# aszepieniec/stark-anatomy

Hardware: AMD Instinct MI355X
Metric: ntt_field_elements_per_sec (higher is better)
Workload: dtype u128; 1 GPU; ntt_fwd_inv_2^20_1gpu; log2n=20, parallelism=single, passes_per_transform=2

## Files before the change

### stark-anatomy_amd/csrc/core.h

```cpp
#pragma once
#include <hip/hip_runtime.h>
#include <dlfcn.h>
#include <cstdio>
#include <cstdlib>
#include <cstring>
#include <algorithm>
#include <atomic>
#include <chrono>
#include <cerrno>
#include <thread>
#include <sys/random.h>
#include <deque>
#include <functional>
#include <future>
#include <map>
#include <mutex>
#include <string>
#include <tuple>
#include <vector>

#pragma GCC visibility push(default)
#include "../../include/starkcore.h"
#pragma GCC visibility pop
#include "ntt_plan.h"

namespace sc { struct FoldIn; }
using namespace sc;

struct sc_vec {
    Fe* d;
    uint64_t n;
    bool owned = true;
};
struct sc_later {
    int slot;
    uint64_t seq;
    hipStream_t st;
};
struct sc_merkle {
    uint64_t* d_levels;
    uint64_t N;
    int logN;
    int slot = -1;
    uint64_t seq = 0;
    hipStream_t st = nullptr;
    bool have_root = false;
    bool lazy = false;
    uint8_t root[64] = {};
};

struct sc_merkle_forest {
    uint64_t* d_levels;
    uint64_t N, count;
    int logN;
    uint64_t* h_roots = nullptr;
    Fe* d_cm = nullptr;
    hipEvent_t done = nullptr;
    hipStream_t st = nullptr;
    bool have_roots = false;
};

namespace sci {

struct DevBuf {
    void* p = nullptr;
    size_t bytes = 0;
};

struct PlanKey {
    int logn;
    uint64_t lo, hi;
    bool operator<(const PlanKey& o) const { return std::tie(logn, lo, hi) < std::tie(o.logn, o.lo, o.hi); }
};
struct PlanTables {
    Fe* mt = nullptr;
    int mt_log = 0;
    Fe* tl = nullptr;
    Fe* th = nullptr;
    Fe* th_ninv = nullptr;
    struct Direct { int logA, logR; bool scaled; Fe* d; };
    std::vector<Direct> direct;
    uint64_t last_use = 0;
};
struct OuterKey {
    uint64_t lo, hi, order, len, batch, col_base;
    int ninv;
    bool operator<(const OuterKey& o) const { return std::tie(lo, hi, order, len, batch, col_base, ninv) < std::tie(o.lo, o.hi, o.order, o.len, o.batch, o.col_base, o.ninv); }
};
struct OuterTable {
    Fe* d = nullptr;
    uint64_t last_use = 0;
};
struct PowKey {
    uint64_t lo, hi, hi_count;
    bool operator<(const PowKey& o) const { return std::tie(lo, hi, hi_count) < std::tie(o.lo, o.hi, o.hi_count); }
};
struct PowTables {
    Fe* lo = nullptr;
    Fe* hi = nullptr;
    uint64_t last_use = 0;
};

struct Ctx {
    bool init = false;
    int device = -1;
    hipStream_t stream = nullptr;
    std::string err;
    NttTuning tuning;
    std::map<PlanKey, PlanTables> plans;
    std::map<PowKey, PowTables> pows;
    std::map<OuterKey, OuterTable> outers;
    uint64_t tick = 0;
    bool foreign_streams = false;
    int small_divisor_direct = 1;
    int div_cols_launch_log = 26;
    int tree_cols_launch_log = 26;
    int eval_chunk_log = 8;
    int eval_points_across_min = 32;
    int eval_across_min_products_log = 26;
    int rescue_tree_split_max_nodes = -1;
    int div_cols_chunk = 0;
    std::vector<hipStream_t> seen_streams;
    DevBuf scratch[8];
    std::map<hipStream_t, DevBuf> ntt_work;
    std::map<hipStream_t, DevBuf> ntt_flags;
    int fast_fixups = 1;
    int num_cus = 256;
    int xcd_remap = 1;
    int fixed_shapes = 1;
    int prio_balance = -1;
    int wave_local = 1;
    unsigned long long* trace = nullptr;
    int forest_four_lane_wgs = 256;
    int merkle_big_nlev = 2;
    int fri_tail = -1;
    int fri_tail_stall = -1;
    size_t verify_stage_bytes = 64ull << 20;
    uint8_t* root_slots = nullptr;
    uint8_t* later_words = nullptr;
    uint64_t root_seq = 0;
    std::vector<int> free_root_slots;
};
constexpr int ROOT_SLOTS = 256;
constexpr size_t ROOT_SLOT_BYTES = 128;
constexpr size_t LATER_WORD_BYTES = 128;
constexpr long SPIN_POLLS = 40000000;

struct PendingFree {
    void* p;
    size_t bytes;
    std::vector<hipEvent_t> evs;
};
#define HIPCHK(expr)                                                                                          \
    do {                                                                                                      \
        hipError_t _e = (expr);                                                                               \
        if (_e != hipSuccess) return fail(SC_ERR_HIP, std::string(#expr) + ": " + hipGetErrorString(_e));     \
    } while (0)

#define SCCHK(expr)              \
    do {                         \
        int _rc = (expr);        \
        if (_rc != SC_OK) return _rc; \
    } while (0)

struct NttOpts {
    uint64_t in_limit = ~0ull;
    const PowTables* coset = nullptr;
    uint32_t cols = 1;
    uint64_t col_stride_in = 0;
};
constexpr uint64_t COLS_ELEMS_PER_LAUNCH = 1ull << 26;
constexpr uint64_t SMALL_DIVISOR = 8;

constexpr uint64_t FUSE_MAX_W = 1ull << 17;

enum BuildMode { BUILD_SYNC = 0, BUILD_ASYNC = 1, BUILD_NOROOT = 2 };

extern Ctx g;
extern std::mutex g_mu;
extern hipStream_t g_comm_stream_for_free;
extern std::future<void> g_rand_worker;
extern size_t g_rand_prefetched;
extern std::multimap<size_t, void*> g_pool;
extern size_t g_pool_bytes, g_pool_cap;
extern std::deque<PendingFree> g_pending;
extern std::vector<hipEvent_t> g_event_pool;

void reap_pending(bool block);
hipError_t pool_alloc(void** p, size_t bytes);
void pool_free(void* p, size_t bytes);
void pool_clear();
hipEvent_t event_get();
int fail(int code, const std::string& msg);
int ensure_init();
int grow_buffer(DevBuf& b, size_t bytes, void** out);
inline int scratch(int slot, size_t bytes, void** out) { return grow_buffer(g.scratch[slot], bytes, out); }
int check_root(Fe root, uint64_t n);
int build_pow_table(Fe** out, uint64_t count, Fe base_m, uint64_t step, Fe scale_m, hipStream_t st);
void free_plans();
int evict_outer_tables();
int get_plan(Fe root, int logn, bool need_ninv, hipStream_t st, PlanTables** out);
inline NttTables tables_of(const PlanTables& t) {
    NttTables tb;
    tb.mt = t.mt; tb.mt_log = t.mt_log; tb.tl = t.tl; tb.th = t.th;
    return tb;
}
int get_pow(Fe base, uint64_t count, hipStream_t st, PowTables** out);
int plan_batched_direct(NttPlanDesc& d, BatchKind kind, int loglen, int logbatch, PlanTables* pt, const Fe* in, Fe* work, Fe* out, BatchExtras ex, hipStream_t st, bool* ok);
int run_plan(NttPlanDesc& d, hipStream_t st);
int ntt_device(const Fe* d_in, Fe* d_out, int logn, Fe root, bool inverse_scale, const NttOpts& o, hipStream_t st);
Fe root_inverse(Fe root, uint64_t n);
int ntt_any(const Fe* d_in, Fe* d_out, uint64_t n, Fe root, bool inverse, const NttOpts& o, hipStream_t st);
int upload(void* d, const void* h, size_t bytes, hipStream_t st);
int download(void* h, const void* d, size_t bytes, hipStream_t st);
int pointwise_div_device(const Fe* a, const Fe* b, Fe* out, uint64_t n, hipStream_t st);
int pointwise_div_enqueue(const Fe* a, const Fe* b, Fe* out, uint64_t n, hipStream_t st, uint32_t* flag);
int gather_device(const Fe* v, const uint64_t* d_idx, uint64_t k, Fe* d_out, hipStream_t st);
int read_small_polled(const void* d_src, size_t bytes, hipStream_t st, void* host_out);
bool upload_small(void* d_dst, const void* host, size_t bytes, hipStream_t st);

int merkle_climb(uint64_t* levels, uint64_t N, int lvl, hipStream_t st, volatile uint64_t* host = nullptr, uint64_t seq = 0, bool* published = nullptr);
int merkle_finish(uint64_t* levels, uint64_t width, hipStream_t st);
int root_slot_get();
int merkle_build_device(const Fe* d_elems, uint64_t N, uint8_t root_out[64], sc_merkle** tree, hipStream_t st, BuildMode mode = BUILD_SYNC, const FoldIn* fold = nullptr);
int merkle_root_wait(sc_merkle* t, bool from_free = false);
void root_poll_unlocked(std::unique_lock<std::mutex>& lk, const sc_merkle* t);
int fold_prepare(const Fe* d_in, uint64_t N, Fe alpha, Fe offset, Fe omega, Fe* d_out, hipStream_t st, FoldIn* f);
int fold_device(const Fe* d_in, uint64_t N, Fe alpha, Fe offset, Fe omega, Fe* d_out, hipStream_t st);
int fold_and_build(const Fe* d_in, uint64_t N, Fe alpha, Fe offset, Fe omega, Fe* d_out, sc_merkle** tree, hipStream_t st);
int fold_constants(uint64_t N, Fe offset, Fe omega, hipStream_t st, PowTables** pw_out, Fe* i2o_m_out);
int host_pool_get(size_t bytes, void** out);
int host_pool_put(void* p);
bool host_pool_holds(const void* p, size_t bytes);
int verify_stage_buffer(size_t bytes, uint8_t** out);

Fe canonical_root(int logn);
Fe ninv_scaled(int logn, int j);
int ntt_cols(const Fe* in, Fe* out, int loglen, int logbatch, bool inverse, hipStream_t st);

constexpr size_t SEEN_STREAMS = 8;
inline hipStream_t pick_stream(void* s) {
    if (s && (hipStream_t)s != g.stream) {
        g.foreign_streams = true;
        hipStream_t st = (hipStream_t)s;
        if (g.seen_streams.size() <= SEEN_STREAMS && std::find(g.seen_streams.begin(), g.seen_streams.end(), st) == g.seen_streams.end())
            g.seen_streams.push_back(st);
    }
    return s ? (hipStream_t)s : g.stream;
}
inline void release_after_streams(void* p, size_t bytes) {
    if (!p) return;
    if (g.seen_streams.size() > SEEN_STREAMS) {
        (void)hipDeviceSynchronize();
        g.seen_streams.clear();
        pool_free(p, bytes);
        return;
    }
    PendingFree f{p, bytes, {}};
    auto mark = [&](hipStream_t st) -> bool {
        if (hipStreamQuery(st) == hipSuccess) return true;
        (void)hipGetLastError();
        hipEvent_t e = event_get();
        if (!e) { (void)hipStreamSynchronize(st); (void)hipGetLastError(); return true; }
        if (hipEventRecord(e, st) != hipSuccess) { (void)hipGetLastError(); g_event_pool.push_back(e); return false; }
        f.evs.push_back(e);
        return true;
    };
    if (g.stream) (void)mark(g.stream);
    if (g_comm_stream_for_free) (void)mark(g_comm_stream_for_free);
    for (size_t i = 0; i < g.seen_streams.size();) {
        if (mark(g.seen_streams[i])) ++i;
        else g.seen_streams.erase(g.seen_streams.begin() + i);
    }
    if (f.evs.empty()) { pool_free(p, bytes); return; }
    g_pending.push_back(std::move(f));
    reap_pending(false);
}
inline Fe fe_from(const uint64_t v[2]) { return Fe{v[0], v[1]}; }
// ... 30 lines not shown
```

### stark-anatomy_amd/csrc/core.hip

```cpp
#include "core.h"


template <int LOGE> struct PassThreads { static constexpr int value = LOGE >= 4 ? 256 : (LOGE == 3 ? 512 : 1024); };

template <int LOGE>
__global__ void __launch_bounds__(PassThreads<LOGE>::value) ntt_pass_kernel(const PassParams P, uint32_t ntiles, int xcd_remap) {
    extern __shared__ __attribute__((aligned(16))) unsigned char smem_raw[];
    Fe* lds = reinterpret_cast<Fe*>(smem_raw);
    uint32_t wg = blockIdx.x, colbits = 0;
    if (P.col_enable) { colbits = (wg >> P.col_tiles_log) << P.col_tiles_log; wg -= colbits; }
    uint32_t tile = wg;
    if (xcd_remap) tile = (wg & 7u) * (ntiles >> 3) + (wg >> 3);
    tile |= colbits;
    Fe* tw = lds + (1u << (P.logR + P.logC));
    tile_twiddles_to_lds(P, P.logR, threadIdx.x, blockDim.x, tw);
    __syncthreads();
    const int nrounds = (P.logR + LOGE - 1) / LOGE;
    int sh = P.logR;
    for (int r = 0; r < nrounds; ++r) {
        const int s = (r == 0) ? (P.logR - LOGE * (nrounds - 1)) : LOGE;
        sh -= s;
        ntt_round_dispatch<LOGE>(P, s, sh, r == 0, tile, threadIdx.x, lds, tw);
        if (r + 1 < nrounds) __syncthreads();
    }
}

constexpr int TRACE_STAMPS = 16;
template <int LOGE, int GLR, int GLC, bool TRACE, bool ALT = false>
__global__ void __launch_bounds__(1 << (GLR + GLC - LOGE)) ntt_pass_kernel_fixed(const PassParams P, uint32_t ntiles, int xcd_remap, int wave_local) {
    extern __shared__ __attribute__((aligned(16))) unsigned char smem_raw[];
    Fe* lds = reinterpret_cast<Fe*>(smem_raw);
    unsigned long long* trow = nullptr;
    if constexpr (TRACE) {
        if (P.trace) {
            trow = P.trace + ((size_t)blockIdx.x * (blockDim.x >> 6) + (threadIdx.x >> 6)) * TRACE_STAMPS;
            if ((threadIdx.x & 63u) == 0) { trow[0] = __builtin_amdgcn_s_memtime(); trow[15] = __builtin_amdgcn_s_memrealtime(); }
        }
    }
    uint32_t wg = blockIdx.x, colbits = 0;
    if (P.col_enable) { colbits = (wg >> P.col_tiles_log) << P.col_tiles_log; wg -= colbits; }
    uint32_t tile = wg;
    if (xcd_remap) tile = (wg & 7u) * (ntiles >> 3) + (wg >> 3);
    tile |= colbits;
    Fe* tw = lds + (1u << (GLR + GLC));
    auto stamp = [&](int i) {
        if constexpr (TRACE) {
            if (trow) {
                if (i == 2) __builtin_amdgcn_s_waitcnt(0);
                if ((threadIdx.x & 63u) == 0 && i < 13) trow[i] = __builtin_amdgcn_s_memtime();
            }
        }
    };
    auto sync = [] { __syncthreads(); };
    auto wsync = [] { __builtin_amdgcn_fence(__ATOMIC_RELEASE, "wavefront"); __builtin_amdgcn_wave_barrier(); __builtin_amdgcn_fence(__ATOMIC_ACQUIRE, "wavefront"); };
    FixedRounds<LOGE, GLR, GLC, 0, ALT>::run(P, tile, threadIdx.x, lds, tw, sync, wsync, stamp, wave_local != 0);
    if constexpr (TRACE) {
        if (trow && (threadIdx.x & 63u) == 0) { __builtin_amdgcn_s_waitcnt(0); trow[14] = __builtin_amdgcn_s_memtime(); trow[13] = __builtin_amdgcn_s_memrealtime(); }
    }
}

template <int GLR, int GLC>
__device__ __forceinline__ uint32_t fixed8_tile(const PassParams& P, uint32_t index, uint32_t ntiles, int xcd_remap) {
    uint32_t wg = index, colbits = 0;
    if (P.col_enable) { colbits = (wg >> P.col_tiles_log) << P.col_tiles_log; wg -= colbits; }
    uint32_t tile = wg;
    if (xcd_remap) tile = (wg & 7u) * (ntiles >> 3) + (wg >> 3);
    return tile | colbits;
}
template <int GLR, int GLC>
__global__ void __launch_bounds__(1 << (GLR + GLC - 3)) __attribute__((amdgpu_waves_per_eu(4)))
ntt_pass_kernel_fixed8(const PassParams P, uint32_t ntiles, int xcd_remap, int wave_local, uint32_t* flags) {
    extern __shared__ __attribute__((aligned(16))) unsigned char smem_raw[];
    Fe* lds = reinterpret_cast<Fe*>(smem_raw);
    const uint32_t tile = fixed8_tile<GLR, GLC>(P, blockIdx.x, ntiles, xcd_remap);
    Fe* tw = lds + (1u << (GLR + GLC));
    auto stamp = [](int) {};
    auto sync = [] { __syncthreads(); };
    auto wsync = [] { __builtin_amdgcn_fence(__ATOMIC_RELEASE, "wavefront"); __builtin_amdgcn_wave_barrier(); __builtin_amdgcn_fence(__ATOMIC_ACQUIRE, "wavefront"); };
    rare_t rare = 0;
    FixedRounds<3, GLR, GLC, 0, false, true>::run(P, tile, threadIdx.x, lds, tw, sync, wsync, stamp, wave_local != 0, rare);
    if (rare_any(rare)) Round<3, 3, GLR, GLC>::store_word_at(flags + blockIdx.x, 0u, 1u);
}

template <int GLR, int GLC>
__global__ void __launch_bounds__(1 << (GLR + GLC - 3)) __attribute__((amdgpu_waves_per_eu(4)))
ntt_pass_redo8_kernel(const PassParams P, uint32_t ntiles, int xcd_remap, int wave_local, uint32_t* flags, int all) {
    extern __shared__ __attribute__((aligned(16))) unsigned char smem_raw[];
    if (!all && flags[blockIdx.x] == 0) return;
    Fe* lds = reinterpret_cast<Fe*>(smem_raw);
    Fe* tw = lds + (1u << (GLR + GLC));
    auto stamp = [](int) {};
    auto sync = [] { __syncthreads(); };
    auto wsync = [] { __builtin_amdgcn_fence(__ATOMIC_RELEASE, "wavefront"); __builtin_amdgcn_wave_barrier(); __builtin_amdgcn_fence(__ATOMIC_ACQUIRE, "wavefront"); };
    FixedRounds<3, GLR, GLC, 0, false>::run(P, fixed8_tile<GLR, GLC>(P, blockIdx.x, ntiles, xcd_remap), threadIdx.x, lds, tw, sync, wsync, stamp, wave_local != 0);
    if (!all) __syncthreads();
    if (threadIdx.x == 0) flags[blockIdx.x] = 0;
}

__global__ void __launch_bounds__(256) pow_table_kernel(Fe* out, uint64_t count, Fe base_m, uint64_t step, Fe scale_m) {
    uint64_t i = (uint64_t)blockIdx.x * blockDim.x + threadIdx.x;
    if (i < count) out[i] = pow_table_entry(base_m, i, step, scale_m);
}

__global__ void __launch_bounds__(256) twiddle_table_kernel(Fe* out, int logB, uint64_t count, uint64_t scale_exp, const Fe* __restrict__ tl, const Fe* __restrict__ th) {
    uint64_t i = (uint64_t)blockIdx.x * blockDim.x + threadIdx.x;
    if (i >= count) return;
    uint64_t k = i >> logB, b = i & ((1ull << logB) - 1);
    out[i] = pow2level(tl, th, b * k * scale_exp);
}

__global__ void __launch_bounds__(256) pointwise_mul_kernel(const Fe* __restrict__ a, const Fe* __restrict__ b, Fe* __restrict__ out, uint64_t n) {
    uint64_t i = (uint64_t)blockIdx.x * blockDim.x + threadIdx.x;
    if (i < n) out[i] = fe_mul(a[i], b[i]);
}

template <int K>
__global__ void __launch_bounds__(256) pointwise_div_kernel(const Fe* __restrict__ a, const Fe* __restrict__ b, Fe* __restrict__ out, uint64_t n, uint32_t* flag) {
    const uint64_t nthreads = (uint64_t)gridDim.x * blockDim.x;
    const uint64_t t = (uint64_t)blockIdx.x * blockDim.x + threadIdx.x;
    Fe bm[K], pre[K];
    Fe acc = fe_mont_one();
    bool zero = false;
#pragma unroll
    for (int k = 0; k < K; ++k) {
        uint64_t i = t + (uint64_t)k * nthreads;
        Fe v = (i < n) ? b[i] : fe_one();
        zero |= fe_is_zero(v);
        bm[k] = to_mont(v);
        pre[k] = acc;
        acc = mont_mul(acc, bm[k]);
    }
    if (zero) atomicOr(flag, 1u);
    Fe inv = mont_inv(acc);
#pragma unroll
    for (int k = K - 1; k >= 0; --k) {
        uint64_t i = t + (uint64_t)k * nthreads;
        Fe ik = mont_mul(inv, pre[k]);
        inv = mont_mul(inv, bm[k]);
        if (i < n) out[i] = mont_mul(a[i], ik);
    }
}

__global__ void __launch_bounds__(256) short_poly_coset_kernel(const Fe* __restrict__ b, uint32_t nb, Fe off_m, const Fe* __restrict__ tl, const Fe* __restrict__ th, Fe* __restrict__ out, uint64_t order) {
    const uint64_t i = (uint64_t)blockIdx.x * blockDim.x + threadIdx.x;
    if (i >= order) return;
    const Fe x_m = mont_mul(off_m, pow2level(tl, th, i));
    Fe acc = b[nb - 1];
    for (uint32_t k = nb - 1; k-- > 0;) acc = fe_add(mont_mul(acc, x_m), b[k]);
    out[i] = acc;
}

__global__ void __launch_bounds__(256) scale_pow_kernel(const Fe* __restrict__ in, Fe* __restrict__ out, uint64_t n, const Fe* __restrict__ lo, const Fe* __restrict__ hi) {
    uint64_t i = (uint64_t)blockIdx.x * blockDim.x + threadIdx.x;
    if (i < n) out[i] = mont_mul(in[i], pow2level(lo, hi, i));
}

__global__ void __launch_bounds__(256) scale_slab_kernel(const Fe* __restrict__ in, Fe* __restrict__ out, uint64_t rows, int logcols, uint64_t row_len, uint64_t col_base,
                                                         const Fe* __restrict__ lo, const Fe* __restrict__ hi) {
    uint64_t t = (uint64_t)blockIdx.x * blockDim.x + threadIdx.x;
    if (t >= (rows << logcols)) return;
    uint64_t r = t >> logcols, c = t & ((1ull << logcols) - 1);
    out[t] = mont_mul(in[t], pow2level(lo, hi, r * row_len + col_base + c));
}

__global__ void __launch_bounds__(256) axpy_shift_kernel(Fe* __restrict__ acc, const Fe* __restrict__ src, uint64_t n_src, uint64_t shift, Fe w_m) {
    uint64_t j = (uint64_t)blockIdx.x * blockDim.x + threadIdx.x;
    if (j >= n_src) return;
    acc[shift + j] = fe_add(acc[shift + j], mont_mul(src[j], w_m));
}

constexpr int DEGREE_PER_THREAD = 4;
constexpr unsigned DEGREE_MAX_BLOCKS = 2048;
constexpr int DEGREE_SLOTS = 8;
__global__ void __launch_bounds__(256) vec_degree_kernel(const Fe* __restrict__ v, uint64_t n, long long* out) {
    const uint64_t step = (uint64_t)gridDim.x * (256 * DEGREE_PER_THREAD);
    long long best = -1;
    for (uint64_t base = (uint64_t)blockIdx.x * (256 * DEGREE_PER_THREAD) + threadIdx.x; base - threadIdx.x < n; base += step) {
        Fe x[DEGREE_PER_THREAD];
#pragma unroll
        for (int k = 0; k < DEGREE_PER_THREAD; ++k) {
            const uint64_t i = base + 256u * k;
            x[k] = i < n ? v[i] : Fe{0, 0};
        }
#pragma unroll
        for (int k = 0; k < DEGREE_PER_THREAD; ++k) {
            const unsigned long long lanes = __ballot(!fe_is_zero(x[k]));
            if (lanes) best = (long long)(base - (threadIdx.x & 63u) + 256u * k + (63 - __clzll((long long)lanes)));
        }
    }
    __shared__ long long wave_best[4];
    if ((threadIdx.x & 63u) == 0) wave_best[threadIdx.x >> 6] = best;
    __syncthreads();
    if (threadIdx.x == 0) {
        long long m = wave_best[0];
#pragma unroll
        for (int w = 1; w < 4; ++w) m = wave_best[w] > m ? wave_best[w] : m;
        if (m >= 0) atomicMax(out + (blockIdx.x & (DEGREE_SLOTS - 1)), m);
    }
}
__global__ void __launch_bounds__(256) vec_degree_cols_kernel(const Fe* __restrict__ v, uint64_t n, uint64_t ld, uint32_t per_col, long long* out) {
    const uint64_t col = blockIdx.x / per_col;
    const uint32_t part = blockIdx.x - (uint32_t)col * per_col;
    const Fe* __restrict__ w = v + col * ld;
    const uint64_t step = (uint64_t)per_col * (256 * DEGREE_PER_THREAD);
    long long best = -1;
    for (uint64_t base = (uint64_t)part * (256 * DEGREE_PER_THREAD) + threadIdx.x; base - threadIdx.x < n; base += step) {
        Fe x[DEGREE_PER_THREAD];
#pragma unroll
        for (int k = 0; k < DEGREE_PER_THREAD; ++k) {
            const uint64_t i = base + 256u * k;
            x[k] = i < n ? w[i] : Fe{0, 0};
        }
#pragma unroll
        for (int k = 0; k < DEGREE_PER_THREAD; ++k) {
            const unsigned long long lanes = __ballot(!fe_is_zero(x[k]));
            if (lanes) best = (long long)(base - (threadIdx.x & 63u) + 256u * k + (63 - __clzll((long long)lanes)));
        }
    }
    __shared__ long long wave_best[4];
    if ((threadIdx.x & 63u) == 0) wave_best[threadIdx.x >> 6] = best;
    __syncthreads();
    if (threadIdx.x == 0) {
        long long m = wave_best[0];
#pragma unroll
        for (int k = 1; k < 4; ++k) m = wave_best[k] > m ? wave_best[k] : m;
        if (m >= 0) atomicMax(out + col, m);
    }
}
static int degree_read(void* fl, hipStream_t st, long long* deg) {
    long long slots[DEGREE_SLOTS];
    SCCHK(read_small_polled(fl, sizeof slots, st, slots));
    long long m = -1;
    for (int i = 0; i < DEGREE_SLOTS; ++i) m = slots[i] > m ? slots[i] : m;
    *deg = m;
// ... 206 lines not shown
    if (const char* sd = getenv("STARKCORE_DEVICE")) dev = atoi(sd) % n;
    HIPCHK(hipSetDevice(dev));
    HIPCHK(hipStreamCreateWithFlags(&g.stream, hipStreamNonBlocking));
    { int cus = 0; if (hipDeviceGetAttribute(&cus, hipDeviceAttributeMultiprocessorCount, dev) == hipSuccess && cus > 0) g.num_cus = cus; }
    { size_t free_b = 0, total_b = 0; if (hipMemGetInfo(&free_b, &total_b) == hipSuccess && total_b) g_pool_cap = total_b / 4; else (void)hipGetLastError(); }
    if (const char* lws = getenv("LOCAL_WORLD_SIZE")) { const int per_dev = (atoi(lws) + n - 1) / n; if (per_dev > 1) g_pool_cap /= (size_t)per_dev; }
    if (const char* cap = getenv("STARKCORE_POOL_CAP_MB")) g_pool_cap = (size_t)atoll(cap) << 20;
    g.device = dev;
    g.init = true;
    return SC_OK;
}

int grow_buffer(DevBuf& b, size_t bytes, void** out) {
    if (b.bytes < bytes) {
        if (b.p) { HIPCHK(hipDeviceSynchronize()); HIPCHK(hipFree(b.p)); b.p = nullptr; b.bytes = 0; }
        size_t want = bytes < (1u << 20) ? (1u << 20) : bytes;
        HIPCHK(hipMalloc(&b.p, want));
        b.bytes = want;
    }
    *out = b.p;
    return SC_OK;
}

int check_root(Fe root, uint64_t n) {
    if (fe_ge_p(root)) return fail(SC_ERR_BAD_ARG, "root is not a canonical residue");
    Fe rm = to_mont(root);
    Fe one = fe_mont_one();
    Fe half = mont_pow(rm, n / 2);
    Fe full = mont_mul(half, half);
    if (!fe_eq(full, one)) return fail(SC_ERR_ROOT_ORDER, "primitive root must be nth root of unity, where n is len(values)");
    if (fe_eq(half, one)) return fail(SC_ERR_ROOT_NOT_PRIMITIVE, "primitive root is not primitive nth root of unity, where n is len(values)");
    return SC_OK;
}

int build_pow_table(Fe** out, uint64_t count, Fe base_m, uint64_t step, Fe scale_m, hipStream_t st) {
    if (count == 0) count = 1;
    HIPCHK(hipMalloc((void**)out, count * sizeof(Fe)));
    unsigned blocks = (unsigned)((count + 255) / 256);
    hipLaunchKernelGGL(pow_table_kernel, dim3(blocks), dim3(256), 0, st, *out, count, base_m, step, scale_m);
    HIPCHK(hipGetLastError());
    return SC_OK;
}

void free_plan_tables(PlanTables& t) {
    hipFree(t.mt); hipFree(t.tl); hipFree(t.th);
    if (t.th_ninv) hipFree(t.th_ninv);
    for (const PlanTables::Direct& e : t.direct) hipFree(e.d);
}

void free_plans() {
    for (auto& kv : g.plans) free_plan_tables(kv.second);
    g.plans.clear();
    for (auto& kv : g.pows) { hipFree(kv.second.lo); hipFree(kv.second.hi); }
    g.pows.clear();
    for (auto& kv : g.outers) hipFree(kv.second.d);
    g.outers.clear();
}

constexpr uint64_t PIN_WINDOW = 64;
constexpr size_t PLAN_CAP = 256, POW_CAP = 64;

template <class Map, class FreeFn>
int evict_tables(Map& m, size_t cap, FreeFn free_entry) {
    if (m.size() < cap) return SC_OK;
    std::vector<std::pair<uint64_t, typename Map::iterator>> old;
    for (auto it = m.begin(); it != m.end(); ++it)
        if (it->second.last_use + PIN_WINDOW < g.tick) old.emplace_back(it->second.last_use, it);
    if (old.empty()) return SC_OK;
    std::sort(old.begin(), old.end(), [](const auto& a, const auto& b) { return a.first < b.first; });
    size_t drop = cap / 4 ? cap / 4 : 1;
    if (drop > old.size()) drop = old.size();
    HIPCHK(hipDeviceSynchronize());
    for (size_t i = 0; i < drop; ++i) { free_entry(old[i].second->second); m.erase(old[i].second); }
    return SC_OK;
}

int get_plan(Fe root, int logn, bool need_ninv, hipStream_t st, PlanTables** out) {
    PlanKey key{logn, root.lo, root.hi};
    auto it = g.plans.find(key);
    bool built = false;
    ++g.tick;
    if (it == g.plans.end()) {
        SCCHK(evict_tables(g.plans, PLAN_CAP, free_plan_tables));
        const uint64_t n = 1ull << logn;
        Fe rm = to_mont(root);
        const TableSizes sz = table_sizes(logn);
        PlanTables t;
        t.mt_log = sz.mt_log;
        SCCHK(build_pow_table(&t.mt, sz.mt, rm, n >> sz.mt_log, fe_mont_one(), st));
        SCCHK(build_pow_table(&t.tl, sz.tl, rm, 1, fe_mont_one(), st));
        SCCHK(build_pow_table(&t.th, sz.th, rm, 4096, fe_mont_one(), st));
        it = g.plans.emplace(key, t).first;
        built = true;
    }
    if (need_ninv && !it->second.th_ninv) {
        const uint64_t n = 1ull << logn;
        Fe ninv_m = mont_inv(to_mont(Fe{n, 0}));
        SCCHK(build_pow_table(&it->second.th_ninv, table_sizes(logn).th, to_mont(root), 4096, ninv_m, st));
        built = true;
    }
    if (built) HIPCHK(hipStreamSynchronize(st));
    it->second.last_use = g.tick;
    *out = &it->second;
    return SC_OK;
}

int get_pow(Fe base, uint64_t count, hipStream_t st, PowTables** out) {
    uint64_t hi_count = (count >> 12) + 1;
    uint64_t hc = 1; while (hc < hi_count) hc <<= 1;
    PowKey key{base.lo, base.hi, hc};
    auto it = g.pows.find(key);
    ++g.tick;
    if (it == g.pows.end()) {
        SCCHK(evict_tables(g.pows, POW_CAP, [](PowTables& t) { hipFree(t.lo); hipFree(t.hi); }));
        Fe bm = to_mont(base);
        PowTables t;
        SCCHK(build_pow_table(&t.lo, 4096, bm, 1, fe_mont_one(), st));
        SCCHK(build_pow_table(&t.hi, hc, bm, 4096, fe_mont_one(), st));
        HIPCHK(hipStreamSynchronize(st));
        it = g.pows.emplace(key, t).first;
    }
    it->second.last_use = g.tick;
    *out = &it->second;
    return SC_OK;
}

int direct_twiddles(PlanTables* pt, const NttPlanDesc& d, int i, bool scaled, hipStream_t st, const Fe** out) {
    const DirectTable t = direct_table(d, i, scaled);
    *out = nullptr;
    if (t.logR + t.logB > g.tuning.direct_tw_max_log) return SC_OK;
    for (const PlanTables::Direct& e : pt->direct)
        if (e.logA == t.logA && e.logR == t.logR && e.scaled == t.scaled) { *out = e.d; return SC_OK; }
    const uint64_t count = 1ull << (t.logR + t.logB);
    Fe* p;
    HIPCHK(hipMalloc((void**)&p, count * sizeof(Fe)));
    pt->direct.push_back({t.logA, t.logR, t.scaled, p});
    hipLaunchKernelGGL(twiddle_table_kernel, dim3((unsigned)((count + 255) / 256)), dim3(256), 0, st, p, t.logB, count, 1ull << t.logA,
                       pt->tl, t.scaled ? pt->th_ninv : pt->th);
    HIPCHK(hipGetLastError());
    HIPCHK(hipStreamSynchronize(st));
    *out = p;
    return SC_OK;
}

int plan_batched_direct(NttPlanDesc& d, BatchKind kind, int loglen, int logbatch, PlanTables* pt, const Fe* in, Fe* work, Fe* out, BatchExtras ex, hipStream_t st, bool* ok) {
    const NttTables tb = tables_of(*pt);
    *ok = plan_batched(d, kind, loglen, logbatch, tb, in, work, out, g.tuning, ex);
    if (!*ok || d.npasses != 2) return SC_OK;
    SCCHK(direct_twiddles(pt, d, 0, false, st, &ex.inner_twd));
    if (ex.inner_twd) *ok = plan_batched(d, kind, loglen, logbatch, tb, in, work, out, g.tuning, ex);
    return SC_OK;
}

int pass_flags(hipStream_t st, uint32_t nwg, uint32_t** out) {
    DevBuf& b = g.ntt_flags[st];
    const void* before = b.p;
    const size_t had = b.bytes;
    void* p;
    SCCHK(grow_buffer(b, (size_t)nwg * sizeof(uint32_t), &p));
    if (p != before || b.bytes != had) HIPCHK(hipMemsetAsync(p, 0, b.bytes, st));
    *out = (uint32_t*)p;
    return SC_OK;
}

template <int LOGE>
int launch_pass(const NttPassDesc& pd, hipStream_t st) {
    int remap = (g.xcd_remap && pd.ntiles >= 16 && (pd.ntiles & 7u) == 0) ? 1 : 0;
    const PassKernel k = pass_kernel(pd, g.fixed_shapes != 0);
    if constexpr (LOGE == 2) {
        if (k.kind == PK_FIXED4) {
            const int lr = pd.p.logR, lc = pd.p.logC;
#define SC_LAUNCH_FIXED(LR, LC, TR, ALT) \
    hipLaunchKernelGGL((ntt_pass_kernel_fixed<2, LR, LC, TR, ALT>), dim3(pd.ntiles * pd.cols), dim3(pd.threads), pd.lds_bytes, st, pd.p, pd.ntiles, remap, g.wave_local)
#define SC_FIXED(LR, LC)                                                          \
            if (lr == LR && lc == LC) {                                           \
                if (k.trace) SC_LAUNCH_FIXED(LR, LC, true, false);                \
                else if (k.alt) SC_LAUNCH_FIXED(LR, LC, false, true);             \
                else SC_LAUNCH_FIXED(LR, LC, false, false);                       \
                return SC_OK;                                                     \
            }
            SC_FIXED4_SHAPES(SC_FIXED)
#undef SC_FIXED
        }
    }
    if constexpr (LOGE == 3) {
        if (k.kind == PK_FIXED8) {
            const int lr = pd.p.logR, lc = pd.p.logC;
            const uint32_t nwg = pd.ntiles * pd.cols;
            const bool fast = g.fast_fixups != 0 && fast_pass_ok(pd.p) && !pass_in_place(pd);
            const int all = (!fast || g.fast_fixups == 2) ? 1 : 0;
            uint32_t* flags;
            SCCHK(pass_flags(st, nwg, &flags));
#define SC_FIXED8(LR, LC)                                                                                                                                   \
            if (lr == LR && lc == LC) {                                                                                                                     \
                if (fast) hipLaunchKernelGGL((ntt_pass_kernel_fixed8<LR, LC>), dim3(nwg), dim3(pd.threads), pd.lds_bytes, st, pd.p, pd.ntiles, remap, g.wave_local, flags); \
                hipLaunchKernelGGL((ntt_pass_redo8_kernel<LR, LC>), dim3(nwg), dim3(pd.threads), pd.lds_bytes, st, pd.p, pd.ntiles, remap, g.wave_local, flags, all); \
                return SC_OK;                                                                                                                               \
            }
            SC_FIXED8_SHAPES(SC_FIXED8)
#undef SC_FIXED8
        }
    }
    hipLaunchKernelGGL(ntt_pass_kernel<LOGE>, dim3(pd.ntiles * pd.cols), dim3(pd.threads), pd.lds_bytes, st, pd.p, pd.ntiles, remap);
    return SC_OK;
}

int run_plan(NttPlanDesc& d, hipStream_t st) {
    size_t trace_off = 0;
    for (int i = 0; i < d.npasses; ++i) {
        d.pass[i].p.prio_balance = pass_prio_balance(d.pass[i], g.prio_balance, g.num_cus);
        d.pass[i].p.trace = g.trace ? g.trace + trace_off : nullptr;
        trace_off += (size_t)d.pass[i].ntiles * d.pass[i].cols * (d.pass[i].threads >> 6) * TRACE_STAMPS;
        switch (d.pass[i].loge) {
            case 1: SCCHK(launch_pass<1>(d.pass[i], st)); break;
            case 2: SCCHK(launch_pass<2>(d.pass[i], st)); break;
            case 3: SCCHK(launch_pass<3>(d.pass[i], st)); break;
            case 4: SCCHK(launch_pass<4>(d.pass[i], st)); break;
            default: return fail(SC_ERR_UNSUPPORTED, "bad loge");
        }
        HIPCHK(hipGetLastError());
    }
    return SC_OK;
}

int ntt_device(const Fe* d_in, Fe* d_out, int logn, Fe root, bool inverse_scale, const NttOpts& o, hipStream_t st) {
    PlanTables* pt;
    SCCHK(get_plan(root, logn, inverse_scale, st, &pt));
    const uint64_t n = 1ull << logn;
    const int m = plan_num_passes(logn, g.tuning);
    NttTables tb = tables_of(*pt);
    tb.th_scaled = (inverse_scale && m > 1) ? pt->th_ninv : nullptr;
    NttIo io;
    io.in = d_in; io.out = d_out; io.in_limit = o.in_limit; io.cols = o.cols; io.col_stride_in = o.col_stride_in;
    if (m > 1) { void* w; SCCHK(grow_buffer(g.ntt_work[st], n * o.cols * sizeof(Fe), &w)); io.work = (Fe*)w; }
    if (o.coset) { io.ol = o.coset->lo; io.oh = o.coset->hi; }
    if (inverse_scale && m == 1) { io.scale_last = true; io.scale = mont_inv(to_mont(Fe{n, 0})); }
    NttPlanDesc d;
    if (!plan_ntt(d, logn, tb, io, g.tuning)) return fail(SC_ERR_UNSUPPORTED, "unsupported transform length");
    if (d.npasses > 1) {
        bool any = false;
        for (int i = 0; i + 1 < d.npasses; ++i) {
            SCCHK(direct_twiddles(pt, d, i, inverse_scale, st, &tb.twd[i]));
            any |= tb.twd[i] != nullptr;
        }
        if (any && !plan_ntt(d, logn, tb, io, g.tuning)) return fail(SC_ERR_UNSUPPORTED, "unsupported transform length");
    }
    return run_plan(d, st);
}

Fe root_inverse(Fe root, uint64_t n) {
    return from_mont(mont_pow(to_mont(root), n - 1));
}

int ntt_any(const Fe* d_in, Fe* d_out, uint64_t n, Fe root, bool inverse, const NttOpts& o, hipStream_t st) {
    if (n <= 1) {
        if (n == 1 && d_in != d_out) HIPCHK(hipMemcpyAsync(d_out, d_in, sizeof(Fe), hipMemcpyDeviceToDevice, st));
        return SC_OK;
    }
    if (!is_pow2(n)) return fail(SC_ERR_NOT_POW2, "cannot compute ntt of non-power-of-two sequence");
    SCCHK(check_root(root, n));
    return ntt_device(d_in, d_out, ilog2(n), inverse ? root_inverse(root, n) : root, inverse, o, st);
}

int upload(void* d, const void* h, size_t bytes, hipStream_t st) {
    if (bytes) HIPCHK(hipMemcpyAsync(d, h, bytes, hipMemcpyHostToDevice, st));
    return SC_OK;
}
int download(void* h, const void* d, size_t bytes, hipStream_t st) {
    if (bytes) HIPCHK(hipMemcpyAsync(h, d, bytes, hipMemcpyDeviceToHost, st));
    HIPCHK(hipStreamSynchronize(st));
    return SC_OK;
}

int pointwise_div_enqueue(const Fe* a, const Fe* b, Fe* out, uint64_t n, hipStream_t st, uint32_t* flag) {
    HIPCHK(hipMemsetAsync(flag, 0, 8, st));
    static const int K = [] { const char* e = getenv("STARKCORE_DIV_K"); return e && atoi(e) == 8 ? 8 : 16; }();
    const uint64_t threads = (n + K - 1) / K;
    const unsigned blocks = (unsigned)((threads + 255) / 256);
    if (K == 8) hipLaunchKernelGGL(pointwise_div_kernel<8>, dim3(blocks), dim3(256), 0, st, a, b, out, n, flag);
    else hipLaunchKernelGGL(pointwise_div_kernel<16>, dim3(blocks), dim3(256), 0, st, a, b, out, n, flag);
    HIPCHK(hipGetLastError());
    return SC_OK;
}
int pointwise_div_device(const Fe* a, const Fe* b, Fe* out, uint64_t n, hipStream_t st) {
    void* fl;
    SCCHK(scratch(4, 256, &fl));
    SCCHK(pointwise_div_enqueue(a, b, out, n, st, (uint32_t*)fl));
    uint64_t hflag = 0;
    SCCHK(read_small_polled(fl, 8, st, &hflag));
    if ((uint32_t)hflag) return fail(SC_ERR_DIV_ZERO, "divide by zero");
    return SC_OK;
}

__global__ void __launch_bounds__(64) words_publish_kernel(const uint64_t* __restrict__ src, uint32_t nwords, volatile uint64_t* host, uint64_t seq) {
    if (threadIdx.x < nwords) host[threadIdx.x] = src[threadIdx.x];
    __threadfence_system();
    if (threadIdx.x == 0) host[8] = seq;
}
int read_small_polled(const void* d_src, size_t bytes, hipStream_t st, void* host_out) {
    const int slot = (bytes <= 64 && ((uintptr_t)d_src & 7) == 0) ? root_slot_get() : -1;
    if (slot < 0) {
        HIPCHK(hipMemcpyAsync(host_out, d_src, bytes, hipMemcpyDeviceToHost, st));
        HIPCHK(hipStreamSynchronize(st));
        return SC_OK;
    }
    const uint64_t seq = ++g.root_seq;
    volatile uint64_t* host = (volatile uint64_t*)(g.root_slots + ROOT_SLOT_BYTES * slot);
    hipLaunchKernelGGL(words_publish_kernel, dim3(1), dim3(64), 0, st, (const uint64_t*)d_src, (uint32_t)((bytes + 7) / 8), host, seq);
    hipError_t e = hipGetLastError();
    bool landed = false;
    if (e == hipSuccess) {
        for (long spin = 0; spin < SPIN_POLLS; ++spin) {
            if (__atomic_load_n(host + 8, __ATOMIC_ACQUIRE) == seq) { landed = true; break; }
            if ((spin & 4095) == 4095) {
                e = hipStreamQuery(st);
                if (e != hipErrorNotReady) break;
                (void)hipGetLastError();
                e = hipSuccess;
            }
        }
        if (!landed) {
            (void)hipGetLastError();
            e = hipStreamSynchronize(st);
            landed = e == hipSuccess && __atomic_load_n(host + 8, __ATOMIC_ACQUIRE) == seq;
            if (e == hipSuccess && !landed) e = hipErrorUnknown;
        }
    }
    if (landed) memcpy(host_out, (const void*)host, bytes);
    else (void)hipStreamSynchronize(st);
    g.free_root_slots.push_back(slot);
    if (!landed) return fail(SC_ERR_HIP, hipGetErrorString(e));
    return SC_OK;
}

static int later_words(int slot, uint32_t** zero_flag, long long** degree_slots) {
    if (!g.later_words) HIPCHK(hipMalloc((void**)&g.later_words, LATER_WORD_BYTES * ROOT_SLOTS));
    uint8_t* w = g.later_words + LATER_WORD_BYTES * slot;
    *degree_slots = (long long*)w;
    *zero_flag = (uint32_t*)(w + DEGREE_SLOTS * sizeof(long long));
    return SC_OK;
}
__global__ void __launch_bounds__(64) divide_flags_publish_kernel(const uint32_t* __restrict__ zero_flag, const long long* __restrict__ degree_slots,
                                                                 volatile uint64_t* host, uint64_t seq) {
    if (threadIdx.x == 0) {
        long long m = -1;
        if (degree_slots) for (int i = 0; i < DEGREE_SLOTS; ++i) m = degree_slots[i] > m ? degree_slots[i] : m;
        host[0] = zero_flag ? (uint64_t)*zero_flag : 0ull;
        host[1] = (uint64_t)m;
        __threadfence_system();
        host[8] = seq;
    }
}
static int divide_flags_later(int slot, const uint32_t* zero_flag, const long long* degree_slots, hipStream_t st, sc_later** out) {
    const uint64_t seq = ++g.root_seq;
    volatile uint64_t* host = (volatile uint64_t*)(g.root_slots + ROOT_SLOT_BYTES * slot);
    hipLaunchKernelGGL(divide_flags_publish_kernel, dim3(1), dim3(64), 0, st, zero_flag, degree_slots, host, seq);
    HIPCHK(hipGetLastError());
    *out = new sc_later{slot, seq, st};
    return SC_OK;
}
static int later_abandon(int slot, hipStream_t st, int rc) {
    (void)hipStreamSynchronize(st);
    g.free_root_slots.push_back(slot);
    return rc;
}
int later_wait(sc_later* h, uint64_t words[8]) {
    volatile uint64_t* host = (volatile uint64_t*)(g.root_slots + ROOT_SLOT_BYTES * h->slot);
    bool landed = false;
    hipError_t e = hipSuccess;
    for (long spin = 0; spin < SPIN_POLLS; ++spin) {
        if (__atomic_load_n(host + 8, __ATOMIC_ACQUIRE) == h->seq) { landed = true; break; }
        if ((spin & 4095) == 4095) {
            e = hipStreamQuery(h->st);
            if (e != hipErrorNotReady) break;
            (void)hipGetLastError();
            e = hipSuccess;
        }
    }
    if (!landed) {
        (void)hipGetLastError();
        e = hipStreamSynchronize(h->st);
        landed = e == hipSuccess && __atomic_load_n(host + 8, __ATOMIC_ACQUIRE) == h->seq;
        if (e == hipSuccess && !landed) e = hipErrorUnknown;
    }
    if (landed) memcpy(words, (const void*)host, 64);
    g.free_root_slots.push_back(h->slot);
    delete h;
    if (!landed) return fail(SC_ERR_HIP, hipGetErrorString(e));
    return SC_OK;
}

int gather_device(const Fe* v, const uint64_t* d_idx, uint64_t k, Fe* d_out, hipStream_t st) {
    hipLaunchKernelGGL(gather_kernel, dim3((unsigned)((k + 255) / 256)), dim3(256), 0, st, v, d_idx, k, d_out);
    HIPCHK(hipGetLastError());
    return SC_OK;
}

int evict_outer_tables() { return evict_tables(g.outers, (size_t)16, [](OuterTable& t) { hipFree(t.d); }); }

}


extern "C" {

int sc_device_count(void) {
    int n = 0;
    if (hipGetDeviceCount(&n) != hipSuccess) return 0;
    return n;
}

int sc_init(int device) {
    std::lock_guard<std::mutex> lk(g_mu);
    if (g.init && (device < 0 || device == g.device)) return SC_OK;
    if (g.init) return fail(SC_ERR_BAD_ARG, "already initialised on another device");
    if (device >= 0) { char buf[16]; snprintf(buf, sizeof buf, "%d", device); setenv("STARKCORE_DEVICE", buf, 1); }
    return ensure_init();
}

int sc_shutdown(void) {
    std::lock_guard<std::mutex> lk(g_mu);
    if (g_rand_worker.valid()) { g_rand_worker.get(); g_rand_prefetched = 0; }
    if (!g.init) return SC_OK;
    hipDeviceSynchronize();
    reap_pending(true);
    for (hipEvent_t e : g_event_pool) (void)hipEventDestroy(e);
    g_event_pool.clear();
    free_plans();
    pool_clear();
    for (auto& b : g.scratch) { if (b.p) hipFree(b.p); b = DevBuf{}; }
    for (auto& kv : g.ntt_work) if (kv.second.p) hipFree(kv.second.p);
    g.ntt_work.clear();
    for (auto& kv : g.ntt_flags) if (kv.second.p) hipFree(kv.second.p);
    g.ntt_flags.clear();
    if (g.later_words) hipFree(g.later_words);
    g.later_words = nullptr;
    if (g.stream) hipStreamDestroy(g.stream);
    g.stream = nullptr;
    g.seen_streams.clear();
    g.foreign_streams = false;
    g.init = false;
    return SC_OK;
}

const char* sc_last_error(void) { return g.err.c_str(); }

int sc_synchronize(void) {
    std::lock_guard<std::mutex> lk(g_mu);
    SCCHK(ensure_init());
    HIPCHK(hipStreamSynchronize(g.stream));
    return SC_OK;
}

int sc_stream(void** stream_out) {
    std::lock_guard<std::mutex> lk(g_mu);
    SCCHK(ensure_init());
    if (!stream_out) return fail(SC_ERR_BAD_ARG, "null argument");
    *stream_out = (void*)g.stream;
    return SC_OK;
}

int sc_stream_join(void* other) {
    std::lock_guard<std::mutex> lk(g_mu);
    SCCHK(ensure_init());
    hipStream_t o = (hipStream_t)other;
    if (o == g.stream) return SC_OK;
    (void)pick_stream(other);
    hipEvent_t a = event_get(), b = event_get();
    if (!a || !b) { if (a) g_event_pool.push_back(a); if (b) g_event_pool.push_back(b); HIPCHK(hipStreamSynchronize(o)); HIPCHK(hipStreamSynchronize(g.stream)); return SC_OK; }
    hipError_t e = hipEventRecord(a, o);
    if (e == hipSuccess) e = hipStreamWaitEvent(g.stream, a, 0);
    if (e == hipSuccess) e = hipEventRecord(b, g.stream);
    if (e == hipSuccess) e = hipStreamWaitEvent(o, b, 0);
    g_event_pool.push_back(a);
    g_event_pool.push_back(b);
    if (e != hipSuccess) return fail(SC_ERR_HIP, hipGetErrorString(e));
    return SC_OK;
}

int sc_set_tuning(const char* key, int value) {
    std::lock_guard<std::mutex> lk(g_mu);
    std::string k(key ? key : "");
    if (k == "max_tile_log") g.tuning.max_tile_log = value;
    else if (k == "loge") g.tuning.loge = value;
    else if (k == "max_col_log") g.tuning.max_col_log = value;
    else if (k == "min_tiles_log") g.tuning.min_tiles_log = value;
    else if (k == "single_pass_max_log") g.tuning.single_pass_max_log = value;
    else if (k == "max_digit_log") g.tuning.max_digit_log = value;
    else if (k == "direct_tw_max_log") g.tuning.direct_tw_max_log = value;
    else if (k == "xcd_remap") g.xcd_remap = value;
    else if (k == "fixed_shapes") g.fixed_shapes = value;
    else if (k == "wave_local") g.wave_local = value;
    else if (k == "fast_fixups") g.fast_fixups = value < 0 ? 0 : (value > 2 ? 2 : value);
    else if (k == "prio_balance") g.prio_balance = value;
    else if (k == "loge_cols") g.tuning.loge_cols = value;
    else if (k == "tw_on_load") g.tuning.tw_on_load = value;
    else if (k == "prune") g.tuning.prune = value;
    else if (k == "merkle_big_nlev") g.merkle_big_nlev = value < 0 ? 0 : (value > 8 ? 8 : value);
    else if (k == "forest_four_lane_wgs") g.forest_four_lane_wgs = value < 0 ? 0 : value;
    else if (k == "fri_tail") g.fri_tail = value ? 1 : 0;
    else if (k == "small_divisor_direct") g.small_divisor_direct = value ? 1 : 0;
    else if (k == "div_cols_chunk") g.div_cols_chunk = value < 0 ? 0 : (value > 65535 ? 65535 : value);
    else if (k == "div_cols_launch_log") g.div_cols_launch_log = value < 1 ? 1 : (value > 26 ? 26 : value);
    else if (k == "tree_cols_launch_log") g.tree_cols_launch_log = value < 1 ? 1 : (value > 26 ? 26 : value);
    else if (k == "eval_chunk_log") g.eval_chunk_log = value < 8 ? 8 : (value > 24 ? 24 : value);
    else if (k == "eval_points_across_min") g.eval_points_across_min = value < 1 ? 1 : value;
    else if (k == "eval_across_min_products_log") g.eval_across_min_products_log = value < 0 ? 0 : (value > 64 ? 64 : value);
    else if (k == "rescue_tree_split_max_nodes") g.rescue_tree_split_max_nodes = value < -1 ? -1 : value;
    else if (k == "verify_stage_kb") g.verify_stage_bytes = (size_t)(value < 16 ? 16 : value) << 10;
    else if (k == "fri_tail_stall") g.fri_tail_stall = value;
    else if (k == "pool_cap_mb") g_pool_cap = (size_t)(value < 0 ? 0 : value) << 20;
    else if (k == "pool_trim") {
        if (g.init) { (void)hipDeviceSynchronize(); reap_pending(true); pool_clear(); }
    }
    else return fail(SC_ERR_BAD_ARG, "unknown tuning key " + k);
    return SC_OK;
}

int sc_ntt_num_passes(uint64_t n) {
    std::lock_guard<std::mutex> lk(g_mu);
    if (n < 2 || !is_pow2(n)) return 0;
    return plan_num_passes(ilog2(n), g.tuning);
}

int sc_debug_trace(void* d_buf) {
    std::lock_guard<std::mutex> lk(g_mu);
    g.trace = (unsigned long long*)d_buf;
    return SC_OK;
}

int sc_vec_alloc(uint64_t n, sc_vec_t** out) {
    std::lock_guard<std::mutex> lk(g_mu);
    SCCHK(ensure_init());
    sc_vec* v = new sc_vec{nullptr, n};
    hipError_t e = pool_alloc((void**)&v->d, (n ? n : 1) * sizeof(Fe));
    if (e != hipSuccess) { delete v; return fail(SC_ERR_HIP, hipGetErrorString(e)); }
    *out = v;
    return SC_OK;
}
int sc_vec_free(sc_vec_t* v) {
    std::lock_guard<std::mutex> lk(g_mu);
    if (!v) return SC_OK;
    if (v->owned) release_after_streams(v->d, (v->n ? v->n : 1) * sizeof(Fe));
    delete v;
    return SC_OK;
}
int sc_vec_wrap(void* d_elems, uint64_t n, sc_vec_t** out) {
    if (!d_elems || !out) return fail(SC_ERR_BAD_ARG, "null argument");
    sc_vec* v = new sc_vec{(Fe*)d_elems, n};
    v->owned = false;
    *out = v;
    return SC_OK;
}
uint64_t sc_vec_len(const sc_vec_t* v) { return v ? v->n : 0; }
void* sc_vec_ptr(sc_vec_t* v) { return v ? v->d : nullptr; }
int sc_vec_zero(sc_vec_t* v) {
    std::lock_guard<std::mutex> lk(g_mu);
    if (!v) return fail(SC_ERR_BAD_ARG, "null vector");
    SCCHK(ensure_init());
    if (v->n) HIPCHK(hipMemsetAsync(v->d, 0, v->n * sizeof(Fe), g.stream));
    return SC_OK;
}
}
namespace sci {
struct SmallPayload { uint64_t w[256]; };
__global__ void __launch_bounds__(256) small_upload_kernel(uint64_t* __restrict__ dst, const SmallPayload p, uint32_t nwords) {
    if (threadIdx.x < nwords) dst[threadIdx.x] = p.w[threadIdx.x];
}
bool upload_small(void* d_dst, const void* host, size_t bytes, hipStream_t st) {
    if (bytes > 4 * sizeof(SmallPayload)) return false;
    const uint8_t* src = (const uint8_t*)host;
    uint64_t* dst = (uint64_t*)d_dst;
    for (size_t left = bytes; left;) {
        const size_t take = left < sizeof(SmallPayload) ? left : sizeof(SmallPayload);
        SmallPayload p;
        p.w[(take - 1) / 8] = 0;
        memcpy(p.w, src, take);
        hipLaunchKernelGGL(small_upload_kernel, dim3(1), dim3(256), 0, st, dst, p, (uint32_t)((take + 7) / 8));
        src += take; dst += (take + 7) / 8; left -= take;
    }
    return hipGetLastError() == hipSuccess;
}
}
extern "C" {
int sc_vec_upload(sc_vec_t* v, uint64_t offset, const void* host, uint64_t count) {
    std::lock_guard<std::mutex> lk(g_mu);
    SCCHK(ensure_init());
    if (!v || offset + count > v->n) return fail(SC_ERR_BAD_ARG, "upload out of range");
    if (count && upload_small(v->d + offset, host, count * sizeof(Fe), g.stream)) return SC_OK;
    SCCHK(upload(v->d + offset, host, count * sizeof(Fe), g.stream));
    HIPCHK(hipStreamSynchronize(g.stream));
    return SC_OK;
}
int sc_vec_download(const sc_vec_t* v, uint64_t offset, void* host, uint64_t count) {
    std::lock_guard<std::mutex> lk(g_mu);
    SCCHK(ensure_init());
    if (!v || offset + count > v->n) return fail(SC_ERR_BAD_ARG, "download out of range");
    return download(host, v->d + offset, count * sizeof(Fe), g.stream);
}
int sc_sample_bytes_dev(const void* bytes, uint64_t count, uint32_t width, void* d_out, void* stream) {
    std::lock_guard<std::mutex> lk(g_mu);
    SCCHK(ensure_init());
    if (!count) return SC_OK;
    if (!bytes || !d_out || width == 0 || width > 32) return fail(SC_ERR_BAD_ARG, "byte strings of 1..32 bytes expected");
    hipStream_t st = pick_stream(stream);
    void* buf;
    SCCHK(scratch(6, count * width + 256, &buf));
    SCCHK(upload(buf, bytes, count * width, st));
    hipLaunchKernelGGL(sample_bytes_kernel, dim3((unsigned)((count + 255) / 256)), dim3(256), 0, st, (const uint8_t*)buf, count, width, (Fe*)d_out);
    HIPCHK(hipGetLastError());
    HIPCHK(hipStreamSynchronize(st));
    return SC_OK;
}
namespace {
uint8_t* g_rand_host = nullptr;
size_t g_rand_host_bytes = 0;
hipEvent_t g_rand_copied = nullptr;
std::atomic<int> g_rand_failed{0};

void rand_fill(size_t bytes) {
    unsigned hw = std::thread::hardware_concurrency();
    size_t nthreads = bytes / (256u << 10);
    if (nthreads > 32) nthreads = 32;
    if (hw && nthreads > hw) nthreads = hw;
    static const long cap = [] { const char* e = getenv("STARKCORE_RAND_THREADS"); return e ? atol(e) : 0L; }();
    if (cap > 0 && nthreads > (size_t)cap) nthreads = (size_t)cap;
    if (nthreads < 1) nthreads = 1;
    auto fill = [](size_t a, size_t b) {
        while (a < b) {
            size_t want = b - a < (1u << 20) ? b - a : (1u << 20);
            ssize_t r = getrandom(g_rand_host + a, want, 0);
            if (r < 0) { if (errno == EINTR) continue; g_rand_failed = 1; return; }
            a += (size_t)r;
        }
    };
    if (nthreads == 1) { fill(0, bytes); return; }
    std::vector<std::thread> pool;
    const size_t per = (bytes + nthreads - 1) / nthreads;
    for (size_t i = 0; i < nthreads; ++i) {
        const size_t a = i * per, b = a + per < bytes ? a + per : bytes;
        if (a < b) pool.emplace_back(fill, a, b);
    }
    for (auto& t : pool) t.join();
}
uint8_t* g_rand_dev = nullptr;
size_t g_rand_dev_bytes = 0;
// ... 568 lines not shown
```

Baseline: 48.86 billion field-elements/s.

## Replace full-grid redo kernel with compacted repair list and small persistent grid

```diff
diff --git a/stark-anatomy_amd/csrc/core.h b/stark-anatomy_amd/csrc/core.h
--- a/stark-anatomy_amd/csrc/core.h
+++ b/stark-anatomy_amd/csrc/core.h
@@ -23,6 +23,7 @@
 #include "../../include/starkcore.h"
 #pragma GCC visibility pop
 #include "ntt_plan.h"
+#include "repair_list.h"
 
 namespace sc { struct FoldIn; }
 using namespace sc;
@@ -124,6 +125,8 @@
     DevBuf scratch[8];
     std::map<hipStream_t, DevBuf> ntt_work;
     std::map<hipStream_t, DevBuf> ntt_flags;
+    std::map<hipStream_t, uint32_t> ntt_flag_seq;
+    int repair_grid = 512;
     int fast_fixups = 1;
     int num_cus = 256;
     int xcd_remap = 1;
diff --git a/stark-anatomy_amd/csrc/core.hip b/stark-anatomy_amd/csrc/core.hip
--- a/stark-anatomy_amd/csrc/core.hip
+++ b/stark-anatomy_amd/csrc/core.hip
@@ -69,7 +69,7 @@
 }
 template <int GLR, int GLC>
 __global__ void __launch_bounds__(1 << (GLR + GLC - 3)) __attribute__((amdgpu_waves_per_eu(4)))
-ntt_pass_kernel_fixed8(const PassParams P, uint32_t ntiles, int xcd_remap, int wave_local, uint32_t* flags) {
+ntt_pass_kernel_fixed8(const PassParams P, uint32_t ntiles, int xcd_remap, int wave_local, const RepairList L) {
     extern __shared__ __attribute__((aligned(16))) unsigned char smem_raw[];
     Fe* lds = reinterpret_cast<Fe*>(smem_raw);
     const uint32_t tile = fixed8_tile<GLR, GLC>(P, blockIdx.x, ntiles, xcd_remap);
@@ -79,7 +79,37 @@
     auto wsync = [] { __builtin_amdgcn_fence(__ATOMIC_RELEASE, "wavefront"); __builtin_amdgcn_wave_barrier(); __builtin_amdgcn_fence(__ATOMIC_ACQUIRE, "wavefront"); };
     rare_t rare = 0;
     FixedRounds<3, GLR, GLC, 0, false, true>::run(P, tile, threadIdx.x, lds, tw, sync, wsync, stamp, wave_local != 0, rare);
-    if (rare_any(rare)) Round<3, 3, GLR, GLC>::store_word_at(flags + blockIdx.x, 0u, 1u);
+    if (rare_any(rare)) {
+        if (__lane_id() == 0) {
+            const uint32_t slot = repair_claim(L, blockIdx.x);
+            if (slot != REPAIR_LOST) Round<3, 3, GLR, GLC>::store_word_at(L.list, slot * 4u, blockIdx.x);
+        }
+    }
+}
+
+template <int GLR, int GLC>
+__global__ void __launch_bounds__(1 << (GLR + GLC - 3)) __attribute__((amdgpu_waves_per_eu(4)))
+ntt_pass_repair8_kernel(const PassParams P, uint32_t ntiles, int xcd_remap, int wave_local, uint32_t nwg, const RepairList L) {
+    extern __shared__ __attribute__((aligned(16))) unsigned char smem_raw[];
+    Fe* lds = reinterpret_cast<Fe*>(smem_raw);
+    Fe* tw = lds + (1u << (GLR + GLC));
+    auto stamp = [](int) {};
+    auto sync = [] { __syncthreads(); };
+    auto wsync = [] { __builtin_amdgcn_fence(__ATOMIC_RELEASE, "wavefront"); __builtin_amdgcn_wave_barrier(); __builtin_amdgcn_fence(__ATOMIC_ACQUIRE, "wavefront"); };
+    const uint32_t entries = __builtin_amdgcn_readfirstlane(repair_entries(L, nwg));
+    if (blockIdx.x == 0 && threadIdx.x == 0) repair_reset_next(L);
+    for (uint32_t trip = 0;; ++trip) {
+        const uint32_t e = repair_entry(blockIdx.x, gridDim.x, trip, entries);
+        if (e >= entries) break;
+        const uint32_t index = __builtin_amdgcn_readfirstlane(L.list[e]);
+        if (index < nwg) {
+            uint32_t tid = threadIdx.x;
+            asm volatile("" : "+v"(tid));
+            FixedRounds<3, GLR, GLC, 0, false>::run(P, fixed8_tile<GLR, GLC>(P, index, ntiles, xcd_remap), tid, lds, tw, sync, wsync, stamp, wave_local != 0);
+            if (threadIdx.x == 0) repair_release(L, index);
+        }
+        __syncthreads();
+    }
 }
 
 template <int GLR, int GLC>
@@ -592,14 +622,22 @@
     return SC_OK;
 }
 
-int pass_flags(hipStream_t st, uint32_t nwg, uint32_t** out) {
+constexpr uint32_t REPAIR_HEAD = 64;
+int pass_flags(hipStream_t st, uint32_t nwg, bool fast, RepairList* out) {
     DevBuf& b = g.ntt_flags[st];
     const void* before = b.p;
     const size_t had = b.bytes;
     void* p;
-    SCCHK(grow_buffer(b, (size_t)nwg * sizeof(uint32_t), &p));
+    SCCHK(grow_buffer(b, (REPAIR_HEAD + 2 * (size_t)nwg) * sizeof(uint32_t), &p));
     if (p != before || b.bytes != had) HIPCHK(hipMemsetAsync(p, 0, b.bytes, st));
-    *out = (uint32_t*)p;
+    uint32_t* words = (uint32_t*)p;
+    const size_t cap = (b.bytes / sizeof(uint32_t) - REPAIR_HEAD) / 2;
+    uint32_t& seq = g.ntt_flag_seq[st];
+    out->flags = words + REPAIR_HEAD;
+    out->list = out->flags + cap;
+    out->count = words + seq % REPAIR_RING;
+    out->next = words + (seq + 1) % REPAIR_RING;
+    if (fast) ++seq;
     return SC_OK;
 }
 
@@ -629,12 +667,18 @@
             const uint32_t nwg = pd.ntiles * pd.cols;
             const bool fast = g.fast_fixups != 0 && fast_pass_ok(pd.p) && !pass_in_place(pd);
             const int all = (!fast || g.fast_fixups == 2) ? 1 : 0;
-            uint32_t* flags;
-            SCCHK(pass_flags(st, nwg, &flags));
+            const uint32_t grid = (uint32_t)g.repair_grid < nwg ? (uint32_t)g.repair_grid : nwg;
+            RepairList rl;
+            SCCHK(pass_flags(st, nwg, fast && !all, &rl));
 #define SC_FIXED8(LR, LC)                                                                                                                                   \
             if (lr == LR && lc == LC) {                                                                                                                     \
-                if (fast) hipLaunchKernelGGL((ntt_pass_kernel_fixed8<LR, LC>), dim3(nwg), dim3(pd.threads), pd.lds_bytes, st, pd.p, pd.ntiles, remap, g.wave_local, flags); \
-                hipLaunchKernelGGL((ntt_pass_redo8_kernel<LR, LC>), dim3(nwg), dim3(pd.threads), pd.lds_bytes, st, pd.p, pd.ntiles, remap, g.wave_local, flags, all); \
+                if (fast) hipLaunchKernelGGL((ntt_pass_kernel_fixed8<LR, LC>), dim3(nwg), dim3(pd.threads), pd.lds_bytes, st, pd.p, pd.ntiles, remap, g.wave_local, rl); \
+                if (all) {                                                                                                                                  \
+                    if (fast) HIPCHK(hipMemsetAsync(rl.count, 0, sizeof(uint32_t), st));                                                                    \
+                    hipLaunchKernelGGL((ntt_pass_redo8_kernel<LR, LC>), dim3(nwg), dim3(pd.threads), pd.lds_bytes, st, pd.p, pd.ntiles, remap, g.wave_local, rl.flags, all); \
+                } else {                                                                                                                                    \
+                    hipLaunchKernelGGL((ntt_pass_repair8_kernel<LR, LC>), dim3(grid), dim3(pd.threads), pd.lds_bytes, st, pd.p, pd.ntiles, remap, g.wave_local, nwg, rl); \
+                }                                                                                                                                           \
                 return SC_OK;                                                                                                                               \
             }
             SC_FIXED8_SHAPES(SC_FIXED8)
@@ -872,6 +916,7 @@
     g.ntt_work.clear();
     for (auto& kv : g.ntt_flags) if (kv.second.p) hipFree(kv.second.p);
     g.ntt_flags.clear();
+    g.ntt_flag_seq.clear();
     if (g.later_words) hipFree(g.later_words);
     g.later_words = nullptr;
     if (g.stream) hipStreamDestroy(g.stream);
@@ -931,6 +976,7 @@
     else if (k == "fixed_shapes") g.fixed_shapes = value;
     else if (k == "wave_local") g.wave_local = value;
     else if (k == "fast_fixups") g.fast_fixups = value < 0 ? 0 : (value > 2 ? 2 : value);
+    else if (k == "repair_grid") g.repair_grid = value < 1 ? 1 : (value > 65536 ? 65536 : value);
     else if (k == "prio_balance") g.prio_balance = value;
     else if (k == "loge_cols") g.tuning.loge_cols = value;
     else if (k == "tw_on_load") g.tuning.tw_on_load = value;
diff --git a/stark-anatomy_amd/csrc/repair_list.h b/stark-anatomy_amd/csrc/repair_list.h
--- /dev/null
+++ b/stark-anatomy_amd/csrc/repair_list.h
@@ -0,0 +1,55 @@
+#pragma once
+#include <stdint.h>
+
+#include "field.cuh"
+
+namespace sc {
+
+constexpr uint32_t REPAIR_RING = 2;
+
+struct RepairList {
+    uint32_t* flags;
+    uint32_t* list;
+    uint32_t* count;
+    uint32_t* next;
+};
+
+SC_HD uint32_t repair_cas(uint32_t* p, uint32_t expect, uint32_t value) {
+#if defined(__HIP_DEVICE_COMPILE__)
+    return atomicCAS(p, expect, value);
+#else
+    const uint32_t old = *p;
+    if (old == expect) *p = value;
+    return old;
+#endif
+}
+SC_HD uint32_t repair_add(uint32_t* p, uint32_t value) {
+#if defined(__HIP_DEVICE_COMPILE__)
+    return atomicAdd(p, value);
+#else
+    const uint32_t old = *p;
+    *p = old + value;
+    return old;
+#endif
+}
+
+constexpr uint32_t REPAIR_LOST = 0xffffffffu;
+SC_HD uint32_t repair_claim(const RepairList& L, uint32_t index) {
+    return repair_cas(L.flags + index, 0u, 1u) == 0u ? repair_add(L.count, 1u) : REPAIR_LOST;
+}
+SC_HD void repair_append(const RepairList& L, uint32_t slot, uint32_t index) { L.list[slot] = index; }
+
+SC_HD uint32_t repair_entries(const RepairList& L, uint32_t nwg) {
+    const uint32_t c = *L.count;
+    return c < nwg ? c : nwg;
+}
+
+SC_HD uint32_t repair_entry(uint32_t wg, uint32_t grid, uint32_t trip, uint32_t entries) {
+    const uint64_t e = (uint64_t)wg + (uint64_t)trip * grid;
+    return e < entries ? (uint32_t)e : entries;
+}
+
+SC_HD void repair_release(const RepairList& L, uint32_t index) { L.flags[index] = 0u; }
+SC_HD void repair_reset_next(const RepairList& L) { *L.next = 0u; }
+
+}
```

New measurement: 49.18 billion field-elements/s, median of 6. No clear change (+0.7%).
